# ppwwyyxx/OpenPano

Hardware: NVIDIA H100
Metric: Mpixels/sec SIFT+match+blend (higher is better)
Workload: dtype f32

## Files before the change

openpano_b200/csrc/engine.cu:

```cuda
#include <mutex>
#include "sift.cuh"
#include <pthread.h>
#include <stdarg.h>
#include <time.h>
#include <stdio.h>
#include <stdlib.h>
#include <string.h>
#include <algorithm>

static thread_local std::string g_create_err;

int ctx_fail(pano_ctx* ctx, int code, const char* fmt, ...) {
  char buf[512];
  va_list ap;
  va_start(ap, fmt);
  vsnprintf(buf, sizeof(buf), fmt, ap);
  va_end(ap);
  if (ctx) ctx->err = buf; else g_create_err = buf;
  return code;
}

int ctx_cuda(pano_ctx* ctx, cudaError_t e, const char* what) {
  return ctx_fail(ctx, PANO_ERR_CUDA, "CUDA error %s (%s) at %s", cudaGetErrorName(e), cudaGetErrorString(e), what);
}
// ... 863 lines not shown
int pano_sift_trace_working_size(const pano_sift_trace* t, int* w0, int* h0) {
  if (t) ctx_enter(t->ctx);
  *w0 = t->wk->h_img[0].w0; *h0 = t->wk->h_img[0].h0;
  return PANO_OK;
}

int pano_sift_trace_octave_size(const pano_sift_trace* t, int o, int* w, int* h) {
  if (t) ctx_enter(t->ctx);
  if (o < 0 || o >= t->wk->n_oct) return PANO_ERR_INVALID;
  *w = t->wk->h_oct[o].w; *h = t->wk->h_oct[o].h;
  return PANO_OK;
}

int pano_sift_trace_plane(pano_sift_trace* t, int kind, int o, int level, float* out) {
  if (t) ctx_enter(t->ctx);
  pano_ctx* ctx = t->ctx;
  SiftWork* wk = t->wk;
  if (kind == 0) {
    const ImgMeta& im = wk->h_img[0];
    return pano_dev_download(ctx, out, wk->arena + im.work_off, (size_t)im.w0 * im.h0 * 3 * sizeof(float));
  }
  if (o < 0 || o >= wk->n_oct) return PANO_ERR_INVALID;
  const OctMeta& om = wk->h_oct[o];
  const float* src = nullptr;
  if (kind == 1 && level >= 0 && level < wk->n_scale) src = wk->arena + om.gauss_off + (size_t)level * om.plane;
  if (kind == 2 && level >= 0 && level < wk->n_scale - 1) src = wk->arena + om.dog_off + (size_t)level * om.plane;
  if (src) {
    PANO_CUDA(ctx, cudaMemcpy2DAsync(out, (size_t)om.w * sizeof(float), src, (size_t)om.pitch * sizeof(float),
                                     (size_t)om.w * sizeof(float), (size_t)om.h, cudaMemcpyDeviceToHost, ctx->stream));
    PANO_CUDA(ctx, cudaStreamSynchronize(ctx->stream));
    return PANO_OK;
  }
  return PANO_ERR_INVALID;
}

int pano_sift_trace_points(pano_sift_trace* t, int stage, int cap, pano_sspoint* out) {
  if (t) ctx_enter(t->ctx);
  pano_ctx* ctx = t->ctx;
  SiftWork* wk = t->wk;
  int n_raw = 0, n_desc = t->fs->h_count[0];
  if (pano_dev_download(ctx, &n_raw, wk->cand_count, sizeof(int))) return PANO_ERR_CUDA;
  n_raw = std::min(n_raw, wk->cap);
  if (stage == 0) {
    std::vector<uint32_t> keys(std::max(n_raw, 1));
    if (n_raw && pano_dev_download(ctx, keys.data(), wk->sorted_keys, n_raw * sizeof(uint32_t))) return PANO_ERR_CUDA;
    for (int i = 0; i < n_raw && i < cap; ++i) {
      memset(&out[i], 0, sizeof(pano_sspoint));
      out[i].pyr_id = keys[i] >> 29; out[i].scale_id = (keys[i] >> 26) & 7;
      out[i].y = (keys[i] >> 13) & 8191; out[i].x = keys[i] & 8191;
    }
    return n_raw;
  }
  std::vector<pano_sspoint> pts(std::max(n_raw, 1));
// ... 45 lines not shown
```

openpano_b200/csrc/sift.cu:

```cuda
#include "sift.cuh"
#include "desc_interval.h"
#include <math.h>
#include <string.h>
#include <algorithm>
#include <cuda.h>

__device__ __forceinline__ void bilinear_coef(int d, float inv, int src_n, int* s, float* frac) {
  float r = ((float)d + 0.5f) * inv - 0.5f;
  int si = (int)floorf(r);
  r -= (float)si;
  if (si < 0) { si = 0; r = 0.f; }
  else if (si + 1 >= src_n) { si = src_n - 2; r = 1.f; }
  *s = si; *frac = r;
}

__global__ void k_working_resize(const ImgMeta* __restrict__ imgs, float* __restrict__ arena) {
  const ImgMeta im = imgs[blockIdx.z];
  int c = blockIdx.x * blockDim.x + threadIdx.x;
  int r = blockIdx.y * blockDim.y + threadIdx.y;
  if (c >= im.w0 || r >= im.h0) return;
  int sx, sy; float rx, ry;
  bilinear_coef(r, im.ifx, im.in_h, &sx, &rx);
  bilinear_coef(c, im.ify, im.in_w, &sy, &ry);
  float irx = 1.0f - rx, iry = 1.0f - ry;
  const float* p0 = im.src + ((size_t)sx * im.in_w + sy) * 3;
  const float* p1 = p0 + (size_t)im.in_w * 3;
  float* dst = arena + im.work_off + ((size_t)r * im.w0 + c) * 3;
#pragma unroll
  for (int ch = 0; ch < 3; ++ch) {
    float p00 = __ldg(p0 + ch), p01 = __ldg(p0 + 3 + ch), p10 = __ldg(p1 + ch), p11 = __ldg(p1 + 3 + ch);
    dst[ch] = rx * (p11 * ry + p10 * iry) + irx * (p01 * ry + p00 * iry);
  }
}

__global__ void k_octave_grey(const ImgMeta* __restrict__ imgs, const OctMeta* __restrict__ octs,
                              float* __restrict__ arena) {
  const OctMeta om = octs[blockIdx.z];
  int c = blockIdx.x * blockDim.x + threadIdx.x;
  int r = blockIdx.y * blockDim.y + threadIdx.y;
  if (c >= om.w || r >= om.h) return;
  const ImgMeta im = imgs[om.img];
  const float* work = arena + im.work_off;
  float v0, v1, v2;
  if (om.oct == 0) {
    const float* p = work + ((size_t)r * im.w0 + c) * 3;
    v0 = p[0]; v1 = p[1]; v2 = p[2];
  } else {
    int sx, sy; float rx, ry;
    bilinear_coef(r, om.ifx, im.h0, &sx, &rx);
    bilinear_coef(c, om.ify, im.w0, &sy, &ry);
    float irx = 1.0f - rx, iry = 1.0f - ry;
    const float* p0 = work + ((size_t)sx * im.w0 + sy) * 3;
    const float* p1 = p0 + (size_t)im.w0 * 3;
    v0 = rx * (p1[3] * ry + p1[0] * iry) + irx * (p0[3] * ry + p0[0] * iry);
    v1 = rx * (p1[4] * ry + p1[1] * iry) + irx * (p0[4] * ry + p0[1] * iry);
    v2 = rx * (p1[5] * ry + p1[2] * iry) + irx * (p0[5] * ry + p0[2] * iry);
  }
  arena[om.gauss_off + (size_t)r * om.pitch + c] = (v0 + v1 + v2) / 3.f;
}

#include "blur_tile.cuh"

__global__ void __launch_bounds__(BT_THREADS)
k_blur_dog(const OctMeta* __restrict__ octs, const int2* __restrict__ span, int n_om,
           float* __restrict__ arena, const __grid_constant__ GaussTable gt) {
  extern __shared__ float smem[];
  const BlurTile tl = find_blur_tile(span, n_om, blockIdx.x);
  const OctMeta om = octs[tl.om];
  const int R = gt.rmax;
  const int GW = BT_W + 2 * R;
  const int GH = BT_H + 2 * R;
  float* grey = smem;
  float* colbuf = smem + GH * GW;
  const int x0 = tl.tx * BT_W, y0 = tl.ty * BT_H;
  const float* g0 = arena + om.gauss_off;
  const int tid = threadIdx.x;

  for (int i = tid; i < GH * GW; i += BT_THREADS) {
    int yy = i / GW, xx = i - yy * GW;
    int gy = min(max(y0 + yy - R, 0), om.h - 1);
    int gx = min(max(x0 + xx - R, 0), om.w - 1);
    grey[i] = __ldg(g0 + (size_t)gy * om.pitch + gx);
  }
  __syncthreads();

  const int tx = tid & (BT_W - 1), ty = tid / BT_W;
  float prev[BT_H / 4];
#pragma unroll
  for (int i = 0; i < BT_H / 4; ++i) prev[i] = grey[(ty + 4 * i + R) * GW + tx + R];

  for (int s = 0; s < gt.nlev; ++s) {
    const int c = gt.center[s];
    const float* taps = gt.taps[s];
    const int cw = BT_W + 2 * c;
    for (int i = tid; i < BT_H * cw; i += BT_THREADS) {
      int y = i / cw, xx = i - y * cw;
      const float* col = grey + (y + R - c) * GW + (xx + R - c);
      float tmp = 0.f;
      for (int k = 0; k <= 2 * c; ++k) tmp += col[k * GW] * taps[k];
      colbuf[y * GW + xx] = tmp;
    }
    __syncthreads();
    float* lvl = arena + om.gauss_off + (size_t)(s + 1) * om.plane;
    float* dog = arena + om.dog_off + (size_t)s * om.plane;
#pragma unroll
    for (int i = 0; i < BT_H / 4; ++i) {
      int y = ty + 4 * i;
      const float* row = colbuf + y * GW + tx;
      float tmp = 0.f;
      for (int k = 0; k <= 2 * c; ++k) tmp += row[k] * taps[k];
      int gx = x0 + tx, gy = y0 + y;
      if (gx < om.w && gy < om.h) {
        size_t o = (size_t)gy * om.pitch + gx;
        lvl[o] = tmp;
        dog[o] = fabsf(prev[i] - tmp);
      }
      prev[i] = tmp;
    }
    __syncthreads();
  }
}

__global__ void __launch_bounds__(BT_THREADS, 3)
k_blur_dog_fast(const OctMeta* __restrict__ octs, const int2* __restrict__ span, int n_om, int n_tiles,
                const TmaDesc* __restrict__ maps, float* __restrict__ arena, const __grid_constant__ GaussTable gt) {
  extern __shared__ __align__(128) float smem[];
  __shared__ __align__(8) uint64_t s_bar[2];
  __shared__ BlurTile s_tile[2];
  const int R = gt.rmax;
  const int RX = (R + 3) & ~3;
  const int GW = BT_W + 2 * RX, GH = BT_H + 2 * R;
  const int GSZ = (GH * GW + 31) & ~31;
  float* grey0 = smem;
  float* colbuf = smem + 2 * GSZ;
  float* outT = colbuf + BLUR_COLBUF_FLOATS(6);
  const int tid = threadIdx.x;
  const uint32_t tile_bytes = (uint32_t)(GH * GW * sizeof(float));
  int t = blockIdx.x;
  if (tid == 0) {
    sbar_init(sm_u32(&s_bar[0]), 1);
    sbar_init(sm_u32(&s_bar[1]), 1);
    asm volatile("fence.mbarrier_init.release.cluster;" ::: "memory");
    if (t < n_tiles) {
      const BlurTile tl = find_blur_tile(span, n_om, t);
      s_tile[0] = tl;
      sbar_expect_tx(sm_u32(&s_bar[0]), tile_bytes);
      tma_load_2d(sm_u32(grey0), maps + tl.om, tl.tx * BT_W - RX, tl.ty * BT_H - R, sm_u32(&s_bar[0]));
    }
  }
  __syncthreads();
  for (int it = 0; t < n_tiles; t += gridDim.x, ++it) {
    const int b = it & 1;
    float* grey = grey0 + b * GSZ;
    const BlurTile tl = s_tile[b];
    const OctMeta om = octs[tl.om];
    const int x0 = tl.tx * BT_W, y0 = tl.ty * BT_H;
    if (tid == 0 && t + (int)gridDim.x < n_tiles) {
      const BlurTile nx = find_blur_tile(span, n_om, t + gridDim.x);
      s_tile[b ^ 1] = nx;
      asm volatile("fence.proxy.async.shared::cta;" ::: "memory");
      sbar_expect_tx(sm_u32(&s_bar[b ^ 1]), tile_bytes);
      tma_load_2d(sm_u32(grey0 + (b ^ 1) * GSZ), maps + nx.om, nx.tx * BT_W - RX, nx.ty * BT_H - R, sm_u32(&s_bar[b ^ 1]));
    }
    sbar_wait(sm_u32(&s_bar[b]), (uint32_t)(it >> 1) & 1u);
    if (x0 - RX < 0 || y0 - R < 0 || x0 + BT_W + RX > om.w || y0 + BT_H + R > om.h) {
      for (int i = tid; i < GH * GW; i += BT_THREADS) {
        const int yy = i / GW, xx = i - yy * GW;
        const int gy = y0 + yy - R, gx = x0 + xx - RX;
        const int cy = min(max(gy, 0), om.h - 1), cx = min(max(gx, 0), om.w - 1);
        if (cy != gy || cx != gx) grey[i] = grey[(cy - y0 + R) * GW + (cx - x0 + RX)];
      }
      __syncthreads();
    }
    const int tx = tid & (BT_W - 1), ty = tid / BT_W;
    const int gx = x0 + tx;
    float prev[BT_H / 4];
#pragma unroll
    for (int i = 0; i < BT_H / 4; ++i) prev[i] = grey[(ty + 4 * i + R) * GW + tx + RX];
    for (int s = 0; s < gt.nlev; ++s) {
      if (gt.center[s] == 3) blur_level<3>(grey, colbuf, outT, gt.taps[s], R, RX, GW, tid);
      else blur_level<6>(grey, colbuf, outT, gt.taps[s], R, RX, GW, tid);
      float* lvl = arena + om.gauss_off + (size_t)(s + 1) * om.plane;
      float* dog = arena + om.dog_off + (size_t)s * om.plane;
#pragma unroll
      for (int i = 0; i < BT_H / 4; ++i) {
        const int y = ty + 4 * i, gy = y0 + y;
        const float v = outT[y * (BT_W + 1) + tx];
        if (gx < om.w && gy < om.h) {
          size_t o = (size_t)gy * om.pitch + gx;
          lvl[o] = v;
          dog[o] = fabsf(prev[i] - v);
        }
        prev[i] = v;
      }
    }
    __syncthreads();
  }
}

__device__ __forceinline__ uint32_t make_key(int oct, int scale, int y, int x) {
  return ((uint32_t)oct << 29) | ((uint32_t)scale << 26) | ((uint32_t)y << 13) | (uint32_t)x;
}

#define EX_ROWS 4
#define EX_LEV 4

__global__ void __launch_bounds__(256)
k_extrema_scan(const OctMeta* __restrict__ octs, const float* __restrict__ arena,
               int nscale, float pre_color_thres, float diff_thres, int cap,
               int* __restrict__ cand_count, uint32_t* __restrict__ cand_keys) {
  const OctMeta om = octs[blockIdx.z];
  const int c = blockIdx.x * 32 + threadIdx.x;
  const int r0 = blockIdx.y * (8 * EX_ROWS) + threadIdx.y + 1;
  if (c < 1 || c >= om.w - 1 || r0 >= om.h - 1) return;
  const float* dog = arena + om.dog_off;
  const int pitch = om.pitch;
  for (int j0 = 1; j0 < nscale - 2; j0 += EX_LEV) {
    float cen[EX_ROWS][EX_LEV];
#pragma unroll
    for (int i = 0; i < EX_ROWS; ++i) {
      const int r = r0 + 8 * i;
#pragma unroll
      for (int l = 0; l < EX_LEV; ++l) {
        const int j = j0 + l;
        cen[i][l] = (r < om.h - 1 && j < nscale - 2) ? __ldg(dog + (size_t)j * om.plane + (size_t)r * pitch + c) : -1.f;
      }
    }
#pragma unroll
    for (int i = 0; i < EX_ROWS; ++i) {
      const int r = r0 + 8 * i;
      const size_t o = (size_t)r * pitch + c;
#pragma unroll
      for (int l = 0; l < EX_LEV; ++l) {
        const float center = cen[i][l];
        const int j = j0 + l;
        if (center < pre_color_thres || r >= om.h - 1 || j >= nscale - 2) continue;
        const float* now = dog + (size_t)j * om.plane;
        float cmp1 = center - diff_thres, cmp2 = center + diff_thres;
        bool mx = true, mn = true;
#pragma unroll
        for (int ds = -1; ds <= 1; ++ds) {
          const float* pl = now + (ptrdiff_t)ds * om.plane;
#pragma unroll
          for (int di = -1; di <= 1; ++di)
#pragma unroll
            for (int dj = -1; dj <= 1; ++dj) {
              if (ds == 0 && di == 0 && dj == 0) continue;
              float v = __ldg(pl + o + (ptrdiff_t)di * pitch + dj);
              if (v >= cmp1) mx = false;
              if (v <= cmp2) mn = false;
            }
        }
        if (mx || mn) {
          int slot = atomicAdd(&cand_count[om.img], 1);
          if (slot < cap) cand_keys[(size_t)om.img * cap + slot] = make_key(om.oct, j, r, c);
        }
      }
    }
  }
}

__global__ void __launch_bounds__(256)
k_rank_sort(const int* __restrict__ cand_count, const uint32_t* __restrict__ keys,
            uint32_t* __restrict__ sorted, int cap) {
  __shared__ uint32_t sk[1024];
  const int img = blockIdx.y;
  const int n = min(cand_count[img], cap);
  const uint32_t* k = keys + (size_t)img * cap;
  for (int c0 = blockIdx.x * 256; c0 < n; c0 += gridDim.x * 256) {
    const int i = c0 + threadIdx.x;
    uint32_t mine = i < n ? k[i] : 0xffffffffu;
    int rank = 0;
    for (int base = 0; base < n; base += 1024) {
      int m = min(1024, n - base);
      __syncthreads();
      for (int t = threadIdx.x; t < m; t += blockDim.x) sk[t] = k[base + t];
      __syncthreads();
      for (int t = 0; t < m; ++t) rank += sk[t] < mine;
    }
    if (i < n) sorted[(size_t)img * cap + rank] = mine;
// ... 85 lines not shown
      for (int k = 0; k < 3; ++k) {
        double l = a[k * 3 + k];
        if (fabs(l) > 1e-6) acc += v[i * 3 + k] * (1.0 / l) * v[j * 3 + k];
      }
      out[i * 3 + j] = acc;
    }
}

struct RefineParams {
  int nscale, depth;
  float offset_thres, contrast_thres, edge_ratio, gauss_sigma, scale_factor;
};

__global__ void k_refine(const OctMeta* __restrict__ octs, const float* __restrict__ arena, int n_oct,
                         const int* __restrict__ cand_count, const uint32_t* __restrict__ sorted,
                         RefineParams rp, int cap, pano_sspoint* __restrict__ out, unsigned char* __restrict__ valid) {
  const int img = blockIdx.y;
  const int n = min(cand_count[img], cap);
  for (int i = blockIdx.x * blockDim.x + threadIdx.x; i < n; i += gridDim.x * blockDim.x) {
  const size_t slot = (size_t)img * cap + i;
  uint32_t key = sorted[slot];
  int oct = key >> 29, s0 = (key >> 26) & 7, y0 = (key >> 13) & 8191, x0 = key & 8191;
  const OctMeta om = octs[img * n_oct + oct];
  const float* dog = arena + om.dog_off;
  const int w = om.w, h = om.h;
#define DG(xx, yy, ss) __ldg(dog + (size_t)(ss) * om.plane + (size_t)(yy) * om.pitch + (xx))
  pano_sspoint sp;
  sp.x = x0; sp.y = y0; sp.pyr_id = oct; sp.scale_id = s0;
  sp.real_x = 0; sp.real_y = 0; sp.dir = 0; sp.scale_factor = 0;
  bool ok = true;
  int nowx = x0, nowy = y0, nows = s0, niter = 0;
  double offset[3] = {0, 0, 0}, delta[3] = {0, 0, 0};
  for (; niter < rp.depth; ++niter) {
    if (!DBETWEEN(nowx, 1, w - 1) || !DBETWEEN(nowy, 1, h - 1) || !DBETWEEN(nows, 1, rp.nscale - 2)) {
      ok = false; break;
    }
    const int x = nowx, y = nowy, s = nows;
    float val = DG(x, y, s);
    delta[0] = (double)((DG(x + 1, y, s) - DG(x - 1, y, s)) / 2);
    delta[1] = (double)((DG(x, y + 1, s) - DG(x, y - 1, s)) / 2);
    delta[2] = (double)((DG(x, y, s + 1) - DG(x, y, s - 1)) / 2);
    double dxx = (double)(DG(x + 1, y, s) + DG(x - 1, y, s) - val - val);
    double dyy = (double)(DG(x, y + 1, s) + DG(x, y - 1, s) - val - val);
    double dss = (double)(DG(x, y, s + 1) + DG(x, y, s - 1) - val - val);
    double dxy = (double)((DG(x + 1, y + 1, s) - DG(x + 1, y - 1, s) - DG(x - 1, y + 1, s) + DG(x - 1, y - 1, s)) / 4);
    double dys = (double)((DG(x, y + 1, s + 1) - DG(x, y - 1, s + 1) - DG(x, y + 1, s - 1) + DG(x, y - 1, s - 1)) / 4);
    double dsx = (double)((DG(x + 1, y, s + 1) - DG(x - 1, y, s + 1) - DG(x + 1, y, s - 1) + DG(x - 1, y, s - 1)) / 4);
    double m[9] = {dxx, dxy, dsx, dxy, dyy, dys, dsx, dys, dss}, inv[9];
    if (!lu3_inverse(m, inv)) sym3_pinv(m, inv);
// ... 765 lines not shown
#define PANO_SQRT1_2_HOST 0.70710678118654752440

int host_gauss_kernel(float sigma, int window_factor, float* taps, int cap) {
  int kw = (int)(ceil(0.3 * (sigma / 2 - 1) + 0.8) * window_factor);
  if (kw % 2 == 0) kw++;
  if (kw > cap) return -kw;
  const int center = kw / 2;
  float* k = taps + center;
  k[0] = 1;
  float exp_coeff = (float)(-1.0 / (sigma * sigma * 2)), wsum = 1;
  for (int i = 1; i <= center; i++) {
    k[i] = expf((float)(i * i) * exp_coeff);
    wsum += k[i] * 2;
  }
  float fac = (float)(1.0 / wsum);
  k[0] = fac;
  for (int i = 1; i <= center; i++) { k[i] *= fac; k[-i] = k[i]; }
  return kw;
}

void sift_work_free(pano_ctx* ctx, SiftWork* wk) {
  if (!wk) return;
  ctx_free(ctx, wk->arena); ctx_free(ctx, wk->d_img); ctx_free(ctx, wk->d_oct); ctx_free(ctx, wk->d_maps); ctx_free(ctx, wk->d_tilespan);
  ctx_free(ctx, wk->cand_count); ctx_free(ctx, wk->cand_keys); ctx_free(ctx, wk->sorted_keys);
  ctx_free(ctx, wk->refined); ctx_free(ctx, wk->kp_valid); ctx_free(ctx, wk->npeaks);
  ctx_free(ctx, wk->dirs); ctx_free(ctx, wk->n_refined);
  ctx_free(ctx, wk->desc_cand); ctx_free(ctx, wk->desc_dir);
  delete wk;
}

typedef CUresult (*tma_encode_fn)(CUtensorMap*, CUtensorMapDataType, cuuint32_t, void*, const cuuint64_t*,
                                  const cuuint64_t*, const cuuint32_t*, const cuuint32_t*, CUtensorMapInterleave,
                                  CUtensorMapSwizzle, CUtensorMapL2promotion, CUtensorMapFloatOOBfill);

int ctx_tma_encode(pano_ctx* ctx, TmaDesc* out, void* base, int rank, const unsigned long long* dims,
                   const unsigned long long* strides_bytes, const unsigned* box) {
  SlowCall sc("ctx_tma_encode");
  if (!ctx->tma_encode) {
    void* fn = nullptr;
    cudaDriverEntryPointQueryResult q;
    cudaError_t e = cudaGetDriverEntryPoint("cuTensorMapEncodeTiled", &fn, cudaEnableDefault, &q);
    if (e != cudaSuccess || q != cudaDriverEntryPointSuccess || !fn)
      return ctx_fail(ctx, PANO_ERR_CUDA, "cuTensorMapEncodeTiled is not available from this driver");
    ctx->tma_encode = fn;
  }
  cuuint64_t gd[5], gs[5];
  cuuint32_t bx[5], es[5];
// ... 9 lines not shown

int sift_run_batch(pano_ctx* ctx, int n, const float* const* d_src, const int* w, const int* h,
                   const pano_params* p, pano_featureset* fs, SiftWork** keep, int cap) {
  if (n <= 0 || !d_src || !w || !h || !p || !fs) return ctx_fail(ctx, PANO_ERR_INVALID, "sift: bad argument");
  if (n > SIFT_MAX_IMG) return ctx_fail(ctx, PANO_ERR_INVALID, "sift: %d images in one batch (limit %d): split the batch", n, SIFT_MAX_IMG);
  const int n_oct = p->num_octave, n_scale = p->num_scale;
  if (n_oct < 1 || n_oct > SIFT_MAX_OCT || n_scale < 4 || n_scale - 1 > SIFT_MAX_LEVELS || n_scale - 2 > 7)
    return ctx_fail(ctx, PANO_ERR_INVALID, "sift: NUM_OCTAVE/NUM_SCALE out of supported range");
  if (cap < 256 || cap > SIFT_CAP_MAX) return ctx_fail(ctx, PANO_ERR_INVALID, "sift: list capacity %d out of range", cap);
  {
    const double sf_max = (double)p->gauss_sigma * std::max(1.0, (double)p->scale_factor);
    const double rad_max = PANO_SQRT1_2_HOST * sf_max * (double)p->desc_hist_scale_factor * 5.0;
    if (!(rad_max <= 127.0))
      return ctx_fail(ctx, PANO_ERR_INVALID, "sift: descriptor windows of up to %.0f pixels radius (limit 127): lower DESC_HIST_SCALE_FACTOR / GAUSS_SIGMA", rad_max);
  }

  SiftWork* wk = new SiftWork;
  wk->n_img = n; wk->n_oct = n_oct; wk->n_scale = n_scale; wk->cap = cap;
  wk->h_img.resize(n);
  wk->h_oct.resize((size_t)n * n_oct);
  size_t off = 0;
  int max_w0 = 0, max_h0 = 0;
  int n_tiles = 0;
  std::vector<int2> tilespan((size_t)n * n_oct);
  for (int i = 0; i < n; ++i) {
    if (w[i] < 2 || h[i] < 2) { delete wk; return ctx_fail(ctx, PANO_ERR_INVALID, "sift: image too small"); }
    ImgMeta& im = wk->h_img[i];
    im.src = d_src[i]; im.in_w = w[i]; im.in_h = h[i];
    float ratio = p->sift_working_size * 2.0f / (w[i] + h[i]);
    im.h0 = (int)(h[i] * ratio); im.w0 = (int)(w[i] * ratio);
    if (im.w0 < 8 || im.h0 < 8 || im.w0 > 8191 || im.h0 > 8191) {
      delete wk; return ctx_fail(ctx, PANO_ERR_INVALID, "sift: working size out of range");
    }
    float fx = (float)im.h0 / h[i], fy = (float)im.w0 / w[i];
    im.ifx = 1.f / fx; im.ify = 1.f / fy;
    im.work_off = (long long)off;
    off += align_up((size_t)im.w0 * im.h0 * 3, 32);
    max_w0 = std::max(max_w0, im.w0); max_h0 = std::max(max_h0, im.h0);
    for (int o = 0; o < n_oct; ++o) {
      OctMeta& om = wk->h_oct[(size_t)i * n_oct + o];
      om.img = i; om.oct = o;
      if (o == 0) { om.w = im.w0; om.h = im.h0; om.ifx = om.ify = 1.f; }
      else {
        float factor = (float)pow((double)p->scale_factor, (double)-o);
        om.w = (int)ceilf(im.w0 * factor); om.h = (int)ceilf(im.h0 * factor);
        if (om.w <= 5 || om.h <= 5) { delete wk; return ctx_fail(ctx, PANO_ERR_INVALID, "sift: octave too small"); }
        float ofx = (float)om.h / im.h0, ofy = (float)om.w / im.w0;
        om.ifx = 1.f / ofx; om.ify = 1.f / ofy;
      }
      om.pitch = (int)align_up((size_t)om.w, 32);
      om.plane = (long long)om.pitch * om.h;
      om.gauss_off = (long long)off; off += (size_t)om.plane * n_scale;
      om.dog_off = (long long)off; off += (size_t)om.plane * (n_scale - 1);
      tilespan[(size_t)i * n_oct + o] = make_int2(n_tiles, ceil_div(om.w, BT_W));
      n_tiles += ceil_div(om.w, BT_W) * ceil_div(om.h, BT_H);
    }
  }
  wk->arena_floats = off;
  wk->n_tiles = n_tiles;

  GaussTable gt;
  memset(&gt, 0, sizeof(gt));
  gt.nlev = n_scale - 1;
  {
    float sigma = p->gauss_sigma;
    for (int s = 0; s < gt.nlev; ++s) {
      int kw = host_gauss_kernel(sigma, p->gauss_window_factor, gt.taps[s], SIFT_MAX_TAPS);
      if (kw < 0) { delete wk; return ctx_fail(ctx, PANO_ERR_INVALID, "sift: gaussian window %d too wide", -kw); }
      gt.center[s] = kw / 2;
      gt.rmax = std::max(gt.rmax, kw / 2);
      sigma *= p->scale_factor;
    }
  }
  bool fast = true;
  for (int s = 0; s < gt.nlev; ++s) fast = fast && (gt.center[s] == 3 || gt.center[s] == 6);

#define SIFT_TRY(call) do { int _rc = (call); if (_rc != 0) { sift_work_free(ctx, wk); return _rc; } } while (0)
#define SIFT_CUDA(call) do { cudaError_t _e = (call); if (_e != cudaSuccess) { int _rc = ctx_cuda(ctx, _e, #call); sift_work_free(ctx, wk); return _rc; } } while (0)

  const size_t nlist = (size_t)n * cap;
  const int n_om = n * n_oct;
  SIFT_TRY(ctx_alloc(ctx, (void**)&wk->arena, off * sizeof(float)));
  SIFT_TRY(ctx_alloc(ctx, (void**)&wk->d_img, n * sizeof(ImgMeta)));
  SIFT_TRY(ctx_alloc(ctx, (void**)&wk->d_oct, wk->h_oct.size() * sizeof(OctMeta)));
  SIFT_TRY(ctx_alloc(ctx, (void**)&wk->d_maps, (size_t)n_om * sizeof(TmaDesc)));
  SIFT_TRY(ctx_alloc(ctx, (void**)&wk->d_tilespan, tilespan.size() * sizeof(int2)));
  SIFT_TRY(ctx_alloc(ctx, (void**)&wk->cand_count, (n + 2) * sizeof(int)));
  SIFT_TRY(ctx_alloc(ctx, (void**)&wk->cand_keys, nlist * sizeof(uint32_t)));
  SIFT_TRY(ctx_alloc(ctx, (void**)&wk->sorted_keys, nlist * sizeof(uint32_t)));
  SIFT_TRY(ctx_alloc(ctx, (void**)&wk->refined, nlist * sizeof(pano_sspoint)));
  SIFT_TRY(ctx_alloc(ctx, (void**)&wk->kp_valid, nlist));
  SIFT_TRY(ctx_alloc(ctx, (void**)&wk->npeaks, nlist * sizeof(int)));
  SIFT_TRY(ctx_alloc(ctx, (void**)&wk->dirs, nlist * SIFT_MAX_PEAKS * sizeof(float)));
  SIFT_TRY(ctx_alloc(ctx, (void**)&wk->n_refined, n * sizeof(int)));
  SIFT_TRY(ctx_alloc(ctx, (void**)&wk->desc_cand, nlist * sizeof(int)));
  SIFT_TRY(ctx_alloc(ctx, (void**)&wk->desc_dir, nlist * sizeof(float)));

  fs->ctx = ctx; fs->n_images = n; fs->cap = cap;
  SIFT_TRY(ctx_alloc(ctx, (void**)&fs->d_desc, nlist * 128 * sizeof(float)));
  SIFT_TRY(ctx_alloc(ctx, (void**)&fs->d_coor, nlist * 4 * sizeof(double)));
  fs->d_real = fs->d_coor + nlist * 2;
  SIFT_TRY(ctx_alloc(ctx, (void**)&fs->d_count, n * sizeof(int)));
  fs->base.resize(n);
  for (int i = 0; i < n; ++i) fs->base[i] = (long long)i * cap;

  {
    void* dsts[4] = {wk->d_img, wk->d_oct, wk->d_tilespan, wk->cand_count};
    const void* srcs[4] = {wk->h_img.data(), wk->h_oct.data(), tilespan.data(), nullptr};
    size_t sizes[4] = {n * sizeof(ImgMeta), wk->h_oct.size() * sizeof(OctMeta), tilespan.size() * sizeof(int2),
                       (n + 2) * sizeof(int)};
    SIFT_TRY(ctx_put_many(ctx, 4, dsts, srcs, sizes));
  }
  if (fast) {
    std::vector<TmaDesc> maps(n_om);
    const int R = gt.rmax;
    for (int k = 0; k < n_om; ++k) {
      const OctMeta& om = wk->h_oct[k];
      unsigned long long dims[2] = {(unsigned long long)om.w, (unsigned long long)om.h};
      unsigned long long strides[1] = {(unsigned long long)om.pitch * sizeof(float)};
      unsigned box[2] = {(unsigned)(BT_W + 2 * ((R + 3) & ~3)), (unsigned)(BT_H + 2 * R)};
      SIFT_TRY(ctx_tma_encode(ctx, &maps[k], wk->arena + om.gauss_off, 2, dims, strides, box));
    }
    SIFT_TRY(ctx_put(ctx, wk->d_maps, maps.data(), maps.size() * sizeof(TmaDesc)));
  }

#define SIFT_LAUNCH(name, kernel, grid, block, smem, ...)                                   \
  do {                                                                                      \
    ctx->launches++;                                                                        \
    if (ctx->profiling) ctx_prof_begin(ctx, name);                                          \
    kernel<<<(grid), (block), (smem), ctx->stream>>>(__VA_ARGS__);                          \
    if (ctx->profiling) ctx_prof_end(ctx);                                                  \
    SIFT_CUDA(cudaGetLastError());                                                          \
  } while (0)

  {
    dim3 b(32, 8), g(ceil_div(max_w0, 32), ceil_div(max_h0, 8), n);
    SIFT_LAUNCH("k_working_resize", k_working_resize, g, b, 0, wk->d_img, wk->arena);
    dim3 g2(ceil_div(max_w0, 32), ceil_div(max_h0, 8), n * n_oct);
    SIFT_LAUNCH("k_octave_grey", k_octave_grey, g2, b, 0, wk->d_img, wk->d_oct, wk->arena);
  }
  {
    const int R = gt.rmax;
    size_t smem = ((size_t)(BT_H + 2 * R) * (BT_W + 2 * R) + (size_t)BT_H * (BT_W + 2 * R)) * sizeof(float);
    if (smem > 200 * 1024) { sift_work_free(ctx, wk); return ctx_fail(ctx, PANO_ERR_INVALID, "sift: blur halo too large"); }
    if (fast) {
      const int GW = BT_W + 2 * ((R + 3) & ~3), GH = BT_H + 2 * R;
      const size_t gsz = ((size_t)GH * GW + 31) & ~(size_t)31;
      size_t smf = (2 * gsz + (size_t)BLUR_COLBUF_FLOATS(6) + (size_t)BT_H * (BT_W + 1)) * sizeof(float);
      SIFT_CUDA(cudaFuncSetAttribute(k_blur_dog_fast, cudaFuncAttributeMaxDynamicSharedMemorySize, (int)smf));
      const int grid = std::min(wk->n_tiles, ctx->num_sms * 3);
      SIFT_LAUNCH("k_blur_dog", k_blur_dog_fast, grid, BT_THREADS, smf, wk->d_oct, wk->d_tilespan, n_om, wk->n_tiles, wk->d_maps,
                  wk->arena, gt);
    } else {
      if (smem > 48 * 1024)
        SIFT_CUDA(cudaFuncSetAttribute(k_blur_dog, cudaFuncAttributeMaxDynamicSharedMemorySize, (int)smem));
      SIFT_LAUNCH("k_blur_dog_generic", k_blur_dog, wk->n_tiles, BT_THREADS, smem, wk->d_oct, wk->d_tilespan, n_om, wk->arena, gt);
    }
  }
  {
    dim3 b(32, 8), g(ceil_div(max_w0 - 1, 32), ceil_div(max_h0 - 2, 8 * EX_ROWS), n * n_oct);
    SIFT_LAUNCH("k_extrema_scan", k_extrema_scan, g, b, 0, wk->d_oct, wk->arena, n_scale, p->pre_color_thres,
                p->judge_extrema_diff_thres, cap, wk->cand_count, wk->cand_keys);
  }
  {
    dim3 g(8, n);
    SIFT_LAUNCH("k_rank_sort", k_rank_sort, g, 256, 0, wk->cand_count, wk->cand_keys, wk->sorted_keys, cap);
    RefineParams rp{n_scale, p->calc_offset_depth, p->offset_thres, p->contrast_thres, p->edge_ratio,
                    p->gauss_sigma, p->scale_factor};
    dim3 g4(16, n);
    SIFT_LAUNCH("k_refine", k_refine, g4, 128, 0, wk->d_oct, wk->arena, n_oct, wk->cand_count, wk->sorted_keys, rp, cap,
                wk->refined, wk->kp_valid);
    const char* ori_env = getenv("PANO_ORI_V1");
    const bool ori_v1 = ori_env && atoi(ori_env) != 0;
    if (ori_v1)
      SIFT_LAUNCH("k_orientation", k_orientation_v1, ctx->num_sms * 8, ORI_WARPS * 32, 0, wk->d_oct, wk->arena, n_oct, n, cap,
                  wk->cand_count, wk->refined, wk->kp_valid, p->ori_radius, p->ori_hist_smooth_count, wk->npeaks, wk->dirs,
                  wk->cand_count + n + 1);
    else
      SIFT_LAUNCH("k_orientation", k_orientation, ctx->num_sms * 8, ORI_WARPS * 32, 0, wk->d_oct, wk->arena, n_oct, n, cap,
                  wk->cand_count, wk->refined, wk->kp_valid, p->ori_radius, p->ori_hist_smooth_count, wk->npeaks, wk->dirs,
                  wk->cand_count + n + 1);
    SIFT_LAUNCH("k_expand_scan", k_expand_scan, n, SCAN_THREADS, 0, wk->cand_count, wk->kp_valid, wk->npeaks,
                wk->dirs, cap, fs->d_count, wk->n_refined, wk->desc_cand, wk->desc_dir);
    DescParams dp{p->desc_hist_scale_factor, p->desc_int_factor};
    const char* desc_env = getenv("PANO_DESC_V1");
// ... 68 lines not shown
```

openpano_b200/csrc/sift.cuh:

```cuda
#pragma once
#include "common.cuh"
#include "match_tc.cuh"

#define SIFT_MAX_OCT 8
#define SIFT_MAX_LEVELS 8
#define SIFT_MAX_TAPS 32
#define SIFT_CAP_DEFAULT 8192
#define SIFT_CAP_MAX (1 << 20)
#define SIFT_MAX_PEAKS 18

struct ImgMeta {
  const float* src;
  int in_w, in_h;
  int w0, h0;
  float ifx, ify;
  long long work_off;
};

struct OctMeta {
  int img, oct;
  int w, h;
  int pitch;
  float ifx, ify;
  long long gauss_off;
  long long dog_off;
  long long plane;
};

struct GaussTable {
  int nlev;
  int rmax;
  int center[SIFT_MAX_LEVELS];
  float taps[SIFT_MAX_LEVELS][SIFT_MAX_TAPS];
};

struct SiftWork {
  int n_img = 0, n_oct = 0, n_scale = 0;
  std::vector<ImgMeta> h_img;
  std::vector<OctMeta> h_oct;
  float* arena = nullptr;
  size_t arena_floats = 0;
  ImgMeta* d_img = nullptr;
  OctMeta* d_oct = nullptr;
  int2* d_tilespan = nullptr;
  TmaDesc* d_maps = nullptr;
  int n_tiles = 0;
  int cap = SIFT_CAP_DEFAULT;
  int* cand_count = nullptr;
  uint32_t* cand_keys = nullptr;
  uint32_t* sorted_keys = nullptr;
  pano_sspoint* refined = nullptr;
  unsigned char* kp_valid = nullptr;
  int* npeaks = nullptr;
  float* dirs = nullptr;
  int* n_desc = nullptr;
  int* n_refined = nullptr;
  int* desc_cand = nullptr;
  float* desc_dir = nullptr;
};

struct pano_featureset {
  pano_ctx* ctx = nullptr;
  int n_images = 0;
  float* d_desc = nullptr;
  double* d_coor = nullptr;
  double* d_real = nullptr;
  int* d_count = nullptr;
  std::vector<long long> base;
  std::vector<int> h_count;
  bool counts_on_host = false;
  cudaEvent_t counts_ready = nullptr;
  unsigned counts_token = 0;
// ... 18 lines not shown
```

Measured before the change: 10410.

## Fuse extrema detection into blur kernel and drop stored DoG planes

The DoG pyramid is no longer written to global memory. The fast blur kernel keeps a three-level DoG ring in shared memory and tests interior tile pixels for extrema in place. Pixels on tile seams are deferred to a small follow-up kernel that recomputes DoG from the Gaussian levels, and refinement does the same. The octave-0 grey conversion is also folded into the resize kernel. This removes DoG write and reread traffic and one full-image pass, at the cost of extra shared memory, lower occupancy risk, seam atomics and recomputing DoG on demand.

Measured after the change: 10850 (median of 6 runs). 1.04x the previous value.

```diff
diff --git a/openpano_b200/csrc/engine.cu b/openpano_b200/csrc/engine.cu
--- a/openpano_b200/csrc/engine.cu
+++ b/openpano_b200/csrc/engine.cu
@@ -909,13 +909,21 @@
   }
   if (o < 0 || o >= wk->n_oct) return PANO_ERR_INVALID;
   const OctMeta& om = wk->h_oct[o];
-  const float* src = nullptr;
-  if (kind == 1 && level >= 0 && level < wk->n_scale) src = wk->arena + om.gauss_off + (size_t)level * om.plane;
-  if (kind == 2 && level >= 0 && level < wk->n_scale - 1) src = wk->arena + om.dog_off + (size_t)level * om.plane;
-  if (src) {
-    PANO_CUDA(ctx, cudaMemcpy2DAsync(out, (size_t)om.w * sizeof(float), src, (size_t)om.pitch * sizeof(float),
+  auto download = [&](float* dst, int lvl) -> int {
+    const float* src = wk->arena + om.gauss_off + (size_t)lvl * om.plane;
+    PANO_CUDA(ctx, cudaMemcpy2DAsync(dst, (size_t)om.w * sizeof(float), src, (size_t)om.pitch * sizeof(float),
                                      (size_t)om.w * sizeof(float), (size_t)om.h, cudaMemcpyDeviceToHost, ctx->stream));
     PANO_CUDA(ctx, cudaStreamSynchronize(ctx->stream));
+    return PANO_OK;
+  };
+  if (kind == 1 && level >= 0 && level < wk->n_scale) return download(out, level);
+  if (kind == 2 && level >= 0 && level < wk->n_scale - 1) {
+    const size_t np = (size_t)om.w * om.h;
+    std::vector<float> next(np);
+    int rc = download(out, level);
+    if (rc == PANO_OK) rc = download(next.data(), level + 1);
+    if (rc != PANO_OK) return rc;
+    for (size_t i = 0; i < np; ++i) out[i] = fabsf(out[i] - next[i]);
     return PANO_OK;
   }
   return PANO_ERR_INVALID;
diff --git a/openpano_b200/csrc/sift.cu b/openpano_b200/csrc/sift.cu
--- a/openpano_b200/csrc/sift.cu
+++ b/openpano_b200/csrc/sift.cu
@@ -14,7 +14,8 @@
   *s = si; *frac = r;
 }
 
-__global__ void k_working_resize(const ImgMeta* __restrict__ imgs, float* __restrict__ arena) {
+__global__ void k_working_resize(const ImgMeta* __restrict__ imgs, const OctMeta* __restrict__ octs, int n_oct,
+                                 float* __restrict__ arena) {
   const ImgMeta im = imgs[blockIdx.z];
   int c = blockIdx.x * blockDim.x + threadIdx.x;
   int r = blockIdx.y * blockDim.y + threadIdx.y;
@@ -26,37 +27,77 @@
   const float* p0 = im.src + ((size_t)sx * im.in_w + sy) * 3;
   const float* p1 = p0 + (size_t)im.in_w * 3;
   float* dst = arena + im.work_off + ((size_t)r * im.w0 + c) * 3;
+  float v[3];
 #pragma unroll
   for (int ch = 0; ch < 3; ++ch) {
     float p00 = __ldg(p0 + ch), p01 = __ldg(p0 + 3 + ch), p10 = __ldg(p1 + ch), p11 = __ldg(p1 + 3 + ch);
-    dst[ch] = rx * (p11 * ry + p10 * iry) + irx * (p01 * ry + p00 * iry);
-  }
-}
-
-__global__ void k_octave_grey(const ImgMeta* __restrict__ imgs, const OctMeta* __restrict__ octs,
+    v[ch] = rx * (p11 * ry + p10 * iry) + irx * (p01 * ry + p00 * iry);
+    dst[ch] = v[ch];
+  }
+  const OctMeta& om = octs[blockIdx.z * n_oct];
+  arena[om.gauss_off + (size_t)r * om.pitch + c] = (v[0] + v[1] + v[2]) / 3.f;
+}
+
+__global__ void k_octave_grey(const ImgMeta* __restrict__ imgs, const OctMeta* __restrict__ octs, int n_oct,
                               float* __restrict__ arena) {
-  const OctMeta om = octs[blockIdx.z];
+  const int img = blockIdx.z / (n_oct - 1), oct = 1 + blockIdx.z % (n_oct - 1);
+  const OctMeta om = octs[img * n_oct + oct];
   int c = blockIdx.x * blockDim.x + threadIdx.x;
   int r = blockIdx.y * blockDim.y + threadIdx.y;
   if (c >= om.w || r >= om.h) return;
-  const ImgMeta im = imgs[om.img];
+  const ImgMeta im = imgs[img];
   const float* work = arena + im.work_off;
-  float v0, v1, v2;
-  if (om.oct == 0) {
-    const float* p = work + ((size_t)r * im.w0 + c) * 3;
-    v0 = p[0]; v1 = p[1]; v2 = p[2];
-  } else {
-    int sx, sy; float rx, ry;
-    bilinear_coef(r, om.ifx, im.h0, &sx, &rx);
-    bilinear_coef(c, om.ify, im.w0, &sy, &ry);
-    float irx = 1.0f - rx, iry = 1.0f - ry;
-    const float* p0 = work + ((size_t)sx * im.w0 + sy) * 3;
-    const float* p1 = p0 + (size_t)im.w0 * 3;
-    v0 = rx * (p1[3] * ry + p1[0] * iry) + irx * (p0[3] * ry + p0[0] * iry);
-    v1 = rx * (p1[4] * ry + p1[1] * iry) + irx * (p0[4] * ry + p0[1] * iry);
-    v2 = rx * (p1[5] * ry + p1[2] * iry) + irx * (p0[5] * ry + p0[2] * iry);
-  }
+  int sx, sy; float rx, ry;
+  bilinear_coef(r, om.ifx, im.h0, &sx, &rx);
+  bilinear_coef(c, om.ify, im.w0, &sy, &ry);
+  float irx = 1.0f - rx, iry = 1.0f - ry;
+  const float* p0 = work + ((size_t)sx * im.w0 + sy) * 3;
+  const float* p1 = p0 + (size_t)im.w0 * 3;
+  const float v0 = rx * (p1[3] * ry + p1[0] * iry) + irx * (p0[3] * ry + p0[0] * iry);
+  const float v1 = rx * (p1[4] * ry + p1[1] * iry) + irx * (p0[4] * ry + p0[1] * iry);
+  const float v2 = rx * (p1[5] * ry + p1[2] * iry) + irx * (p0[5] * ry + p0[2] * iry);
   arena[om.gauss_off + (size_t)r * om.pitch + c] = (v0 + v1 + v2) / 3.f;
+}
+
+struct ExtremaParams {
+  int nscale;
+  float pre_color_thres, diff_thres;
+  int cap;
+  int* cand_count;
+  uint32_t* cand_keys;
+  int seam_cap;
+  int* seam_count;
+  uint32_t* seam_keys;
+};
+
+__device__ __forceinline__ uint32_t make_key(int oct, int scale, int y, int x) {
+  return ((uint32_t)oct << 29) | ((uint32_t)scale << 26) | ((uint32_t)y << 13) | (uint32_t)x;
+}
+
+template <class DoG>
+__device__ __forceinline__ bool is_extremum(float center, float pre_color_thres, float diff_thres, const DoG& dog) {
+  if (center < pre_color_thres) return false;
+  const float cmp1 = center - diff_thres, cmp2 = center + diff_thres;
+  bool mx = true, mn = true;
+#pragma unroll
+  for (int ds = -1; ds <= 1; ++ds) {
+#pragma unroll
+    for (int di = -1; di <= 1; ++di)
+#pragma unroll
+      for (int dj = -1; dj <= 1; ++dj) {
+        if (ds == 0 && di == 0 && dj == 0) continue;
+        const float v = dog(ds, di, dj);
+        if (v >= cmp1) mx = false;
+        if (v <= cmp2) mn = false;
+      }
+    if (!mx && !mn) return false;
+  }
+  return true;
+}
+
+__device__ __forceinline__ void append_candidate(const ExtremaParams& ep, int img, uint32_t key) {
+  const int slot = atomicAdd(&ep.cand_count[img], 1);
+  if (slot < ep.cap) ep.cand_keys[(size_t)img * ep.cap + slot] = key;
 }
 
 #include "blur_tile.cuh"
@@ -85,10 +126,6 @@
   __syncthreads();
 
   const int tx = tid & (BT_W - 1), ty = tid / BT_W;
-  float prev[BT_H / 4];
-#pragma unroll
-  for (int i = 0; i < BT_H / 4; ++i) prev[i] = grey[(ty + 4 * i + R) * GW + tx + R];
-
   for (int s = 0; s < gt.nlev; ++s) {
     const int c = gt.center[s];
     const float* taps = gt.taps[s];
@@ -102,7 +139,6 @@
     }
     __syncthreads();
     float* lvl = arena + om.gauss_off + (size_t)(s + 1) * om.plane;
-    float* dog = arena + om.dog_off + (size_t)s * om.plane;
 #pragma unroll
     for (int i = 0; i < BT_H / 4; ++i) {
       int y = ty + 4 * i;
@@ -110,20 +146,17 @@
       float tmp = 0.f;
       for (int k = 0; k <= 2 * c; ++k) tmp += row[k] * taps[k];
       int gx = x0 + tx, gy = y0 + y;
-      if (gx < om.w && gy < om.h) {
-        size_t o = (size_t)gy * om.pitch + gx;
-        lvl[o] = tmp;
-        dog[o] = fabsf(prev[i] - tmp);
-      }
-      prev[i] = tmp;
+      if (gx < om.w && gy < om.h) lvl[(size_t)gy * om.pitch + gx] = tmp;
     }
     __syncthreads();
   }
 }
 
+#define EX_RING_FLOATS (3 * BT_H * BT_W)
 __global__ void __launch_bounds__(BT_THREADS, 3)
-k_blur_dog_fast(const OctMeta* __restrict__ octs, const int2* __restrict__ span, int n_om, int n_tiles,
-                const TmaDesc* __restrict__ maps, float* __restrict__ arena, const __grid_constant__ GaussTable gt) {
+k_blur_extrema(const OctMeta* __restrict__ octs, const int2* __restrict__ span, int n_om, int n_tiles,
+               const TmaDesc* __restrict__ maps, float* __restrict__ arena, const __grid_constant__ GaussTable gt,
+               const ExtremaParams ep) {
   extern __shared__ __align__(128) float smem[];
   __shared__ __align__(8) uint64_t s_bar[2];
   __shared__ BlurTile s_tile[2];
@@ -134,6 +167,7 @@
   float* grey0 = smem;
   float* colbuf = smem + 2 * GSZ;
   float* outT = colbuf + BLUR_COLBUF_FLOATS(6);
+  float* ring = outT + BT_H * (BT_W + 1);
   const int tid = threadIdx.x;
   const uint32_t tile_bytes = (uint32_t)(GH * GW * sizeof(float));
   int t = blockIdx.x;
@@ -174,6 +208,8 @@
     }
     const int tx = tid & (BT_W - 1), ty = tid / BT_W;
     const int gx = x0 + tx;
+    const bool col_in = gx >= 1 && gx <= om.w - 2;
+    const bool col_seam = tx == 0 || tx == BT_W - 1;
     float prev[BT_H / 4];
 #pragma unroll
     for (int i = 0; i < BT_H / 4; ++i) prev[i] = grey[(ty + 4 * i + R) * GW + tx + RX];
@@ -181,81 +217,89 @@
       if (gt.center[s] == 3) blur_level<3>(grey, colbuf, outT, gt.taps[s], R, RX, GW, tid);
       else blur_level<6>(grey, colbuf, outT, gt.taps[s], R, RX, GW, tid);
       float* lvl = arena + om.gauss_off + (size_t)(s + 1) * om.plane;
-      float* dog = arena + om.dog_off + (size_t)s * om.plane;
+      float* dog = ring + (s % 3) * (BT_H * BT_W);
 #pragma unroll
       for (int i = 0; i < BT_H / 4; ++i) {
         const int y = ty + 4 * i, gy = y0 + y;
         const float v = outT[y * (BT_W + 1) + tx];
-        if (gx < om.w && gy < om.h) {
-          size_t o = (size_t)gy * om.pitch + gx;
-          lvl[o] = v;
-          dog[o] = fabsf(prev[i] - v);
-        }
+        if (gx < om.w && gy < om.h) lvl[(size_t)gy * om.pitch + gx] = v;
+        dog[y * BT_W + tx] = fabsf(prev[i] - v);
         prev[i] = v;
       }
+      if (s >= 2) {
+        __syncthreads();
+        const int j = s - 1;
+        const float* d0 = ring + ((s - 2) % 3) * (BT_H * BT_W);
+        const float* d1 = ring + ((s - 1) % 3) * (BT_H * BT_W);
+        const float* d2 = dog;
+#pragma unroll 1
+        for (int i = 0; i < BT_H / 4; ++i) {
+          const int y = ty + 4 * i, gy = y0 + y;
+          if (!col_in || gy < 1 || gy > om.h - 2) continue;
+          const int o = y * BT_W + tx;
+          const float center = d1[o];
+          if (center < ep.pre_color_thres) continue;
+          if (col_seam || y == 0 || y == BT_H - 1) {
+            const int slot = atomicAdd(&ep.seam_count[om.img], 1);
+            if (slot < ep.seam_cap) ep.seam_keys[(size_t)om.img * ep.seam_cap + slot] = make_key(om.oct, j, gy, gx);
+            continue;
+          }
+          auto at = [&](int ds, int di, int dj) {
+            const float* d = ds < 0 ? d0 : ds == 0 ? d1 : d2;
+            return d[o + di * BT_W + dj];
+          };
+          if (is_extremum(center, ep.pre_color_thres, ep.diff_thres, at))
+            append_candidate(ep, om.img, make_key(om.oct, j, gy, gx));
+        }
+      }
     }
     __syncthreads();
   }
 }
 
-__device__ __forceinline__ uint32_t make_key(int oct, int scale, int y, int x) {
-  return ((uint32_t)oct << 29) | ((uint32_t)scale << 26) | ((uint32_t)y << 13) | (uint32_t)x;
-}
-
-#define EX_ROWS 4
-#define EX_LEV 4
+__device__ __forceinline__ void test_from_levels(const ExtremaParams& ep, const OctMeta& om, const float* arena,
+                                                 int j, int gy, int gx, float center) {
+  const float* c = arena + om.gauss_off + (size_t)gy * om.pitch + gx;
+  auto at = [&](int ds, int di, int dj) {
+    const float* q = c + (ptrdiff_t)(j + ds) * om.plane + (ptrdiff_t)di * om.pitch + dj;
+    return fabsf(__ldg(q) - __ldg(q + om.plane));
+  };
+  if (is_extremum(center, ep.pre_color_thres, ep.diff_thres, at))
+    append_candidate(ep, om.img, make_key(om.oct, j, gy, gx));
+}
 
 __global__ void __launch_bounds__(256)
-k_extrema_scan(const OctMeta* __restrict__ octs, const float* __restrict__ arena,
-               int nscale, float pre_color_thres, float diff_thres, int cap,
-               int* __restrict__ cand_count, uint32_t* __restrict__ cand_keys) {
-  const OctMeta om = octs[blockIdx.z];
-  const int c = blockIdx.x * 32 + threadIdx.x;
-  const int r0 = blockIdx.y * (8 * EX_ROWS) + threadIdx.y + 1;
-  if (c < 1 || c >= om.w - 1 || r0 >= om.h - 1) return;
-  const float* dog = arena + om.dog_off;
-  const int pitch = om.pitch;
-  for (int j0 = 1; j0 < nscale - 2; j0 += EX_LEV) {
-    float cen[EX_ROWS][EX_LEV];
+k_extrema_seams(const OctMeta* __restrict__ octs, int n_oct, const float* __restrict__ arena, const ExtremaParams ep) {
+  const int img = blockIdx.y;
+  const int n = min(ep.seam_count[img], ep.seam_cap);
+  for (int i = blockIdx.x * blockDim.x + threadIdx.x; i < n; i += gridDim.x * blockDim.x) {
+    const uint32_t key = ep.seam_keys[(size_t)img * ep.seam_cap + i];
+    const int oct = key >> 29, j = (key >> 26) & 7, gy = (key >> 13) & 8191, gx = key & 8191;
+    const OctMeta om = octs[img * n_oct + oct];
+    const float* c = arena + om.gauss_off + (size_t)gy * om.pitch + gx;
+    test_from_levels(ep, om, arena, j, gy, gx, fabsf(__ldg(c + (size_t)j * om.plane) - __ldg(c + (size_t)(j + 1) * om.plane)));
+  }
+}
+
+#define EXS_THREADS 192
+
+__global__ void __launch_bounds__(EXS_THREADS, 6)
+k_extrema_scan(const OctMeta* __restrict__ octs, const int2* __restrict__ span, int n_om,
+               const float* __restrict__ arena, const ExtremaParams ep) {
+  const BlurTile tl = find_blur_tile(span, n_om, blockIdx.x);
+  const OctMeta om = octs[tl.om];
+  const int x0 = tl.tx * BT_W, y0 = tl.ty * BT_H;
+  for (int p = threadIdx.x; p < BT_W * BT_H; p += EXS_THREADS) {
+    const int gx = x0 + (p & (BT_W - 1)), gy = y0 + p / BT_W;
+    if (gx < 1 || gx > om.w - 2 || gy < 1 || gy > om.h - 2) continue;
+    const float* c = arena + om.gauss_off + (size_t)gy * om.pitch + gx;
+    float lv[SIFT_MAX_LEVELS];
 #pragma unroll
-    for (int i = 0; i < EX_ROWS; ++i) {
-      const int r = r0 + 8 * i;
+    for (int l = 1; l < SIFT_MAX_LEVELS; ++l) lv[l] = l <= ep.nscale - 2 ? __ldg(c + (size_t)l * om.plane) : 0.f;
 #pragma unroll
-      for (int l = 0; l < EX_LEV; ++l) {
-        const int j = j0 + l;
-        cen[i][l] = (r < om.h - 1 && j < nscale - 2) ? __ldg(dog + (size_t)j * om.plane + (size_t)r * pitch + c) : -1.f;
-      }
-    }
-#pragma unroll
-    for (int i = 0; i < EX_ROWS; ++i) {
-      const int r = r0 + 8 * i;
-      const size_t o = (size_t)r * pitch + c;
-#pragma unroll
-      for (int l = 0; l < EX_LEV; ++l) {
-        const float center = cen[i][l];
-        const int j = j0 + l;
-        if (center < pre_color_thres || r >= om.h - 1 || j >= nscale - 2) continue;
-        const float* now = dog + (size_t)j * om.plane;
-        float cmp1 = center - diff_thres, cmp2 = center + diff_thres;
-        bool mx = true, mn = true;
-#pragma unroll
-        for (int ds = -1; ds <= 1; ++ds) {
-          const float* pl = now + (ptrdiff_t)ds * om.plane;
-#pragma unroll
-          for (int di = -1; di <= 1; ++di)
-#pragma unroll
-            for (int dj = -1; dj <= 1; ++dj) {
-              if (ds == 0 && di == 0 && dj == 0) continue;
-              float v = __ldg(pl + o + (ptrdiff_t)di * pitch + dj);
-              if (v >= cmp1) mx = false;
-              if (v <= cmp2) mn = false;
-            }
-        }
-        if (mx || mn) {
-          int slot = atomicAdd(&cand_count[om.img], 1);
-          if (slot < cap) cand_keys[(size_t)om.img * cap + slot] = make_key(om.oct, j, r, c);
-        }
-      }
+    for (int j = 1; j < SIFT_MAX_LEVELS - 1; ++j) {
+      if (j >= ep.nscale - 2) break;
+      test_from_levels(ep, om, arena, j, gy, gx, fabsf(lv[j] - lv[j + 1]));
     }
   }
 }
@@ -387,9 +431,13 @@
   uint32_t key = sorted[slot];
   int oct = key >> 29, s0 = (key >> 26) & 7, y0 = (key >> 13) & 8191, x0 = key & 8191;
   const OctMeta om = octs[img * n_oct + oct];
-  const float* dog = arena + om.dog_off;
+  const float* gauss = arena + om.gauss_off;
   const int w = om.w, h = om.h;
-#define DG(xx, yy, ss) __ldg(dog + (size_t)(ss) * om.plane + (size_t)(yy) * om.pitch + (xx))
+  auto dog_at = [&](int xx, int yy, int ss) {
+    const float* q = gauss + (size_t)ss * om.plane + (size_t)yy * om.pitch + xx;
+    return fabsf(__ldg(q) - __ldg(q + om.plane));
+  };
+#define DG(xx, yy, ss) dog_at(xx, yy, ss)
   pano_sspoint sp;
   sp.x = x0; sp.y = y0; sp.pyr_id = oct; sp.scale_id = s0;
   sp.real_x = 0; sp.real_y = 0; sp.dir = 0; sp.scale_factor = 0;
@@ -1201,7 +1249,7 @@
 void sift_work_free(pano_ctx* ctx, SiftWork* wk) {
   if (!wk) return;
   ctx_free(ctx, wk->arena); ctx_free(ctx, wk->d_img); ctx_free(ctx, wk->d_oct); ctx_free(ctx, wk->d_maps); ctx_free(ctx, wk->d_tilespan);
-  ctx_free(ctx, wk->cand_count); ctx_free(ctx, wk->cand_keys); ctx_free(ctx, wk->sorted_keys);
+  ctx_free(ctx, wk->cand_count); ctx_free(ctx, wk->cand_keys); ctx_free(ctx, wk->seam_keys); ctx_free(ctx, wk->sorted_keys);
   ctx_free(ctx, wk->refined); ctx_free(ctx, wk->kp_valid); ctx_free(ctx, wk->npeaks);
   ctx_free(ctx, wk->dirs); ctx_free(ctx, wk->n_refined);
   ctx_free(ctx, wk->desc_cand); ctx_free(ctx, wk->desc_dir);
@@ -1257,6 +1305,7 @@
   size_t off = 0;
   int max_w0 = 0, max_h0 = 0;
   int n_tiles = 0;
+  size_t seam_cap = 0;
   std::vector<int2> tilespan((size_t)n * n_oct);
   for (int i = 0; i < n; ++i) {
     if (w[i] < 2 || h[i] < 2) { delete wk; return ctx_fail(ctx, PANO_ERR_INVALID, "sift: image too small"); }
@@ -1272,6 +1321,7 @@
     im.work_off = (long long)off;
     off += align_up((size_t)im.w0 * im.h0 * 3, 32);
     max_w0 = std::max(max_w0, im.w0); max_h0 = std::max(max_h0, im.h0);
+    size_t img_tiles = 0;
     for (int o = 0; o < n_oct; ++o) {
       OctMeta& om = wk->h_oct[(size_t)i * n_oct + o];
       om.img = i; om.oct = o;
@@ -1286,10 +1336,11 @@
       om.pitch = (int)align_up((size_t)om.w, 32);
       om.plane = (long long)om.pitch * om.h;
       om.gauss_off = (long long)off; off += (size_t)om.plane * n_scale;
-      om.dog_off = (long long)off; off += (size_t)om.plane * (n_scale - 1);
       tilespan[(size_t)i * n_oct + o] = make_int2(n_tiles, ceil_div(om.w, BT_W));
       n_tiles += ceil_div(om.w, BT_W) * ceil_div(om.h, BT_H);
-    }
+      img_tiles += (size_t)ceil_div(om.w, BT_W) * ceil_div(om.h, BT_H);
+    }
+    seam_cap = std::max(seam_cap, img_tiles * (2 * BT_W + 2 * (BT_H - 2)) * (size_t)(n_scale - 3));
   }
   wk->arena_floats = off;
   wk->n_tiles = n_tiles;
@@ -1320,7 +1371,8 @@
   SIFT_TRY(ctx_alloc(ctx, (void**)&wk->d_oct, wk->h_oct.size() * sizeof(OctMeta)));
   SIFT_TRY(ctx_alloc(ctx, (void**)&wk->d_maps, (size_t)n_om * sizeof(TmaDesc)));
   SIFT_TRY(ctx_alloc(ctx, (void**)&wk->d_tilespan, tilespan.size() * sizeof(int2)));
-  SIFT_TRY(ctx_alloc(ctx, (void**)&wk->cand_count, (n + 2) * sizeof(int)));
+  SIFT_TRY(ctx_alloc(ctx, (void**)&wk->cand_count, (2 * n + 2) * sizeof(int)));
+  SIFT_TRY(ctx_alloc(ctx, (void**)&wk->seam_keys, (size_t)n * seam_cap * sizeof(uint32_t)));
   SIFT_TRY(ctx_alloc(ctx, (void**)&wk->cand_keys, nlist * sizeof(uint32_t)));
   SIFT_TRY(ctx_alloc(ctx, (void**)&wk->sorted_keys, nlist * sizeof(uint32_t)));
   SIFT_TRY(ctx_alloc(ctx, (void**)&wk->refined, nlist * sizeof(pano_sspoint)));
@@ -1343,7 +1395,7 @@
     void* dsts[4] = {wk->d_img, wk->d_oct, wk->d_tilespan, wk->cand_count};
     const void* srcs[4] = {wk->h_img.data(), wk->h_oct.data(), tilespan.data(), nullptr};
     size_t sizes[4] = {n * sizeof(ImgMeta), wk->h_oct.size() * sizeof(OctMeta), tilespan.size() * sizeof(int2),
-                       (n + 2) * sizeof(int)};
+                       (2 * n + 2) * sizeof(int)};
     SIFT_TRY(ctx_put_many(ctx, 4, dsts, srcs, sizes));
   }
   if (fast) {
@@ -1370,32 +1422,39 @@
 
   {
     dim3 b(32, 8), g(ceil_div(max_w0, 32), ceil_div(max_h0, 8), n);
-    SIFT_LAUNCH("k_working_resize", k_working_resize, g, b, 0, wk->d_img, wk->arena);
-    dim3 g2(ceil_div(max_w0, 32), ceil_div(max_h0, 8), n * n_oct);
-    SIFT_LAUNCH("k_octave_grey", k_octave_grey, g2, b, 0, wk->d_img, wk->d_oct, wk->arena);
+    SIFT_LAUNCH("k_working_resize", k_working_resize, g, b, 0, wk->d_img, wk->d_oct, n_oct, wk->arena);
+    if (n_oct > 1) {
+      int max_w1 = 0, max_h1 = 0;
+      for (int i = 0; i < n; ++i) {
+        max_w1 = std::max(max_w1, wk->h_oct[(size_t)i * n_oct + 1].w);
+        max_h1 = std::max(max_h1, wk->h_oct[(size_t)i * n_oct + 1].h);
+      }
+      dim3 g2(ceil_div(max_w1, 32), ceil_div(max_h1, 8), n * (n_oct - 1));
+      SIFT_LAUNCH("k_octave_grey", k_octave_grey, g2, b, 0, wk->d_img, wk->d_oct, n_oct, wk->arena);
+    }
   }
   {
+    const ExtremaParams ep{n_scale, p->pre_color_thres, p->judge_extrema_diff_thres, cap, wk->cand_count, wk->cand_keys,
+                           (int)seam_cap, wk->cand_count + n + 2, wk->seam_keys};
     const int R = gt.rmax;
     size_t smem = ((size_t)(BT_H + 2 * R) * (BT_W + 2 * R) + (size_t)BT_H * (BT_W + 2 * R)) * sizeof(float);
     if (smem > 200 * 1024) { sift_work_free(ctx, wk); return ctx_fail(ctx, PANO_ERR_INVALID, "sift: blur halo too large"); }
     if (fast) {
       const int GW = BT_W + 2 * ((R + 3) & ~3), GH = BT_H + 2 * R;
       const size_t gsz = ((size_t)GH * GW + 31) & ~(size_t)31;
-      size_t smf = (2 * gsz + (size_t)BLUR_COLBUF_FLOATS(6) + (size_t)BT_H * (BT_W + 1)) * sizeof(float);
-      SIFT_CUDA(cudaFuncSetAttribute(k_blur_dog_fast, cudaFuncAttributeMaxDynamicSharedMemorySize, (int)smf));
+      size_t smf = (2 * gsz + (size_t)BLUR_COLBUF_FLOATS(6) + (size_t)BT_H * (BT_W + 1) + EX_RING_FLOATS) * sizeof(float);
+      SIFT_CUDA(cudaFuncSetAttribute(k_blur_extrema, cudaFuncAttributeMaxDynamicSharedMemorySize, (int)smf));
       const int grid = std::min(wk->n_tiles, ctx->num_sms * 3);
-      SIFT_LAUNCH("k_blur_dog", k_blur_dog_fast, grid, BT_THREADS, smf, wk->d_oct, wk->d_tilespan, n_om, wk->n_tiles, wk->d_maps,
-                  wk->arena, gt);
+      SIFT_LAUNCH("k_blur_extrema", k_blur_extrema, grid, BT_THREADS, smf, wk->d_oct, wk->d_tilespan, n_om, wk->n_tiles,
+                  wk->d_maps, wk->arena, gt, ep);
+      SIFT_LAUNCH("k_extrema_seams", k_extrema_seams, dim3(8, n), 256, 0, wk->d_oct, n_oct, wk->arena, ep);
     } else {
       if (smem > 48 * 1024)
         SIFT_CUDA(cudaFuncSetAttribute(k_blur_dog, cudaFuncAttributeMaxDynamicSharedMemorySize, (int)smem));
       SIFT_LAUNCH("k_blur_dog_generic", k_blur_dog, wk->n_tiles, BT_THREADS, smem, wk->d_oct, wk->d_tilespan, n_om, wk->arena, gt);
-    }
-  }
-  {
-    dim3 b(32, 8), g(ceil_div(max_w0 - 1, 32), ceil_div(max_h0 - 2, 8 * EX_ROWS), n * n_oct);
-    SIFT_LAUNCH("k_extrema_scan", k_extrema_scan, g, b, 0, wk->d_oct, wk->arena, n_scale, p->pre_color_thres,
-                p->judge_extrema_diff_thres, cap, wk->cand_count, wk->cand_keys);
+      SIFT_LAUNCH("k_extrema_scan", k_extrema_scan, wk->n_tiles, EXS_THREADS, 0, wk->d_oct, wk->d_tilespan, n_om,
+                  wk->arena, ep);
+    }
   }
   {
     dim3 g(8, n);
diff --git a/openpano_b200/csrc/sift.cuh b/openpano_b200/csrc/sift.cuh
--- a/openpano_b200/csrc/sift.cuh
+++ b/openpano_b200/csrc/sift.cuh
@@ -23,7 +23,6 @@
   int pitch;
   float ifx, ify;
   long long gauss_off;
-  long long dog_off;
   long long plane;
 };
 
@@ -48,6 +47,7 @@
   int cap = SIFT_CAP_DEFAULT;
   int* cand_count = nullptr;
   uint32_t* cand_keys = nullptr;
+  uint32_t* seam_keys = nullptr;
   uint32_t* sorted_keys = nullptr;
   pano_sspoint* refined = nullptr;
   unsigned char* kp_valid = nullptr;
```
